# FireMines/zk_stark_project

Hardware: NVIDIA B200
Metric: stark_proofs_per_sec (higher is better)
Workload: dtype u128 mod p (f128 field, 4x u32 limbs), u32 BLAKE3

## Files before the change

### zk_stark_project_b200/csrc/kernels.cuh

```cuda
#pragma once
#include "f128.cuh"
#include "blake3.cuh"
#include "coin.cuh"

namespace zkb {

struct PowTab {
    const fe* lo;
    const fe* hi;
    uint32_t l1;
};
__device__ __forceinline__ fe powtab(const PowTab& t, uint32_t e) {
    fe a = fe_ldg(t.lo + (e & ((1u << t.l1) - 1u)));
    fe b = fe_ldg(t.hi + (e >> t.l1));
    return fe_mul(a, b);
}

struct LdeMat {
    fe* data;
    uint32_t log_n, log_beta, w, log_p;
    uint32_t log_shard, bw, bw_magic, view, q_self;
    uint64_t blk_stride;
    uint32_t k0, log_kc;
};
__device__ __forceinline__ uint32_t lde_full_log_p(const LdeMat& m) { return m.log_p + m.log_shard; }
__device__ __forceinline__ size_t lde_row_base(const LdeMat& m, uint32_t k, uint32_t i) {
    const uint32_t lt = m.log_n - lde_full_log_p(m);
    const uint32_t t_low = i & ((1u << lt) - 1u), slot = i >> lt;
    const size_t panel = ((size_t)(k - m.k0) << lt) + t_low;
    const size_t np = (size_t)1 << (m.log_kc + lt);
    const uint32_t chunk = m.view == 0 ? (slot >> m.log_p) : 0u;
    return (((size_t)chunk * np + panel) * m.bw << m.log_p) + (slot & ((1u << m.log_p) - 1u));
}
__device__ __forceinline__ size_t lde_col_off(const LdeMat& m, uint32_t j) {
    const uint32_t blk = (j * m.bw_magic) >> 16;
    return (size_t)blk * m.blk_stride + ((size_t)(j - blk * m.bw) << m.log_p);
}
__device__ __forceinline__ size_t lde_addr(const LdeMat& m, uint32_t k, uint32_t i, uint32_t j) {
    return lde_row_base(m, k, i) + lde_col_off(m, j);
}

__global__ void k_transpose_cols(const fe* __restrict__ in, fe* __restrict__ out, uint32_t n, uint32_t wc, uint32_t out_stride) {
    __shared__ uint4 tile[32][33];
    const uint32_t i0 = blockIdx.x * 32, j0 = blockIdx.y * 32;
    for (uint32_t jj = threadIdx.y; jj < 32; jj += blockDim.y) {
        uint32_t j = j0 + jj, i = i0 + threadIdx.x;
        if (j < wc && i < n) {
            const fe v = fe_canon(fe_load(in + (size_t)j * n + i), 0);
            tile[jj][threadIdx.x] = make_uint4(v.x[0], v.x[1], v.x[2], v.x[3]);
        }
    }
    __syncthreads();
    for (uint32_t ii = threadIdx.y; ii < 32; ii += blockDim.y) {
        uint32_t i = i0 + ii, j = j0 + threadIdx.x;
        if (j < wc && i < n) reinterpret_cast<uint4*>(out)[(size_t)i * out_stride + j] = tile[threadIdx.x][ii];
    }
}

struct NttPass {
    const fe* in;
    fe* out;
    uint32_t log_n, a, b;
    uint32_t w_in, w_out;
    uint32_t col0_in, col0_out, ncols, cj;
    uint32_t n_cosets, coset0;
    uint64_t in_coset_stride, out_coset_stride;
    uint32_t coset;
    uint32_t inverse;
    uint32_t log_tab;
    uint32_t log_lde;
    uint32_t out_panel;
    uint32_t log_shard;
    uint32_t panel_k0, log_kc;
    uint32_t do_scale;
    fe scale;
    PowTab roots;
    const fe* pow3;
    const fe* tw_tab;
};

__device__ __forceinline__ uint32_t bitrev(uint32_t v, uint32_t bits) { return bits == 0 ? 0u : (__brev(v) >> (32 - bits)); }

template <int RHO, int NC>
__device__ __forceinline__ void ntt_unit(fe* __restrict__ col, const uint32_t rs, const uint32_t cstride, const fe4* __restrict__ tw,
                                         const uint32_t base, const uint32_t lam0) {
    constexpr int R = 1 << RHO;
    fe x[NC][R];
    const uint32_t step = rs << lam0;
    fe* p = col + base * rs;
#pragma unroll
    for (int c = 0; c < NC; c++)
#pragma unroll
        for (int d = 0; d < R; d++) x[c][d] = p[d * step + c * cstride];
    const uint32_t base_low = base & ((1u << lam0) - 1u);
#pragma unroll
    for (int s = 0; s < RHO; s++) {
        const fe4* twl = tw + ((1u << (lam0 + s)) - 1u) + base_low;
#pragma unroll
        for (int t = 0; t < (1 << s); t++) {
            const fe4 w = twl[(uint32_t)t << lam0];
#pragma unroll
            for (int g = 0; g < (R >> (s + 1)); g++) {
                const int d0 = g * (2 << s) + t, d1 = d0 + (1 << s);
#pragma unroll
                for (int c = 0; c < NC; c++) {
                    const fe u = x[c][d0];
                    const fe v = fe_mul_pre4(x[c][d1], w);
                    x[c][d0] = fe_add(u, v);
                    x[c][d1] = fe_sub(u, v);
                }
            }
        }
    }
#pragma unroll
    for (int c = 0; c < NC; c++)
#pragma unroll
        for (int d = 0; d < R; d++) p[d * step + c * cstride] = x[c][d];
}

__device__ __forceinline__ fe ntt_twiddle(const NttPass& p, uint32_t k, uint32_t t_low, uint32_t q) {
    const uint32_t logS = p.b - p.a;
    const uint32_t tab_mask = (1u << p.log_tab) - 1u;
    const uint32_t lam = 32 - __clz(q + 1);
    const uint32_t th = q + 1 - (1u << (lam - 1));
    const uint32_t l = p.a + lam;
    (void)logS;
    uint32_t e = (t_low << (p.log_tab - l)) + (th << (p.log_tab - lam));
    if (p.coset) e += (k << (p.log_n - l)) << (p.log_tab - p.log_lde);
    e &= tab_mask;
    if (p.inverse) e = (0u - e) & tab_mask;
    fe t = powtab(p.roots, e);
    if (p.coset) t = fe_mul(t, fe_ldg(p.pow3 + l));
    return t;
}
__global__ void k_build_twiddles(const NttPass p, fe* __restrict__ table) {
    const uint32_t S = 1u << (p.b - p.a);
    const uint64_t total = ((uint64_t)p.n_cosets << p.a) * (S - 1u);
    const uint64_t id = (uint64_t)blockIdx.x * blockDim.x + threadIdx.x;
    if (id >= total) return;
    const uint32_t q = (uint32_t)(id % (S - 1u));
    const uint32_t tile = (uint32_t)(id / (S - 1u));
    fe_store(table + id, ntt_twiddle(p, tile >> p.a, tile & ((1u << p.a) - 1u), q));
}

template <int RHO>
__device__ __forceinline__ void ntt_unit_plain(fe* __restrict__ col, const uint32_t rs, const fe* __restrict__ tw, const uint32_t base, const uint32_t lam0) {
    constexpr int R = 1 << RHO;
    fe x[R];
    const uint32_t step = rs << lam0;
    fe* p = col + base * rs;
#pragma unroll
    for (int d = 0; d < R; d++) x[d] = p[d * step];
    const uint32_t base_low = base & ((1u << lam0) - 1u);
#pragma unroll
    for (int s = 0; s < RHO; s++) {
        const fe* twl = tw + ((1u << (lam0 + s)) - 1u) + base_low;
#pragma unroll
        for (int t = 0; t < (1 << s); t++) {
            const fe w = twl[(uint32_t)t << lam0];
#pragma unroll
            for (int g = 0; g < (R >> (s + 1)); g++) {
                const int d0 = g * (2 << s) + t, d1 = d0 + (1 << s);
                const fe u = x[d0];
                const fe v = fe_mul(x[d1], w);
                x[d0] = fe_add(u, v);
                x[d1] = fe_sub(u, v);
            }
        }
    }
#pragma unroll
    for (int d = 0; d < R; d++) p[d * step] = x[d];
}
template <int RHO>
__device__ __forceinline__ void ntt_round_plain(fe* sm, const fe* tw, uint32_t rs, uint32_t log_cj, uint32_t logS, uint32_t lam0) {
    const uint32_t cj_mask = (1u << log_cj) - 1u;
    const uint32_t units = (1u << (logS - RHO)) << log_cj;
    for (uint32_t idx = threadIdx.x; idx < units; idx += blockDim.x) {
        const uint32_t jj = idx & cj_mask, u = idx >> log_cj;
        const uint32_t base = (u & ((1u << lam0) - 1u)) + ((u >> lam0) << (lam0 + RHO));
        ntt_unit_plain<RHO>(sm + jj, rs, tw, base, lam0);
    }
}
__device__ __forceinline__ void ntt_rounds_plain(fe* sm, const fe* tw, uint32_t rs, uint32_t log_cj, uint32_t logS) {
    for (uint32_t lam0 = 0; lam0 < logS;) {
        const uint32_t left = logS - lam0;
        if (left >= 3 && left != 4) { ntt_round_plain<3>(sm, tw, rs, log_cj, logS, lam0); lam0 += 3; }
        else if (left >= 2) { ntt_round_plain<2>(sm, tw, rs, log_cj, logS, lam0); lam0 += 2; }
        else { ntt_round_plain<1>(sm, tw, rs, log_cj, logS, lam0); lam0 += 1; }
        __syncthreads();
    }
}

template <int RHO, int NC>
__device__ __forceinline__ void ntt_round(fe* sm, const fe4* tw, uint32_t rs, uint32_t log_cj, uint32_t logS, uint32_t lam0) {
    const uint32_t log_cw = log_cj - (NC == 2 ? 1u : 0u);
    const uint32_t cw_mask = (1u << log_cw) - 1u;
    const uint32_t units = (1u << (logS - RHO)) << log_cw;
    for (uint32_t idx = threadIdx.x; idx < units; idx += blockDim.x) {
        const uint32_t jj = idx & cw_mask, u = idx >> log_cw;
        const uint32_t base = (u & ((1u << lam0) - 1u)) + ((u >> lam0) << (lam0 + RHO));
        ntt_unit<RHO, NC>(sm + jj, rs, 1u << log_cw, tw, base, lam0);
    }
}
template <int NC>
__device__ __forceinline__ void ntt_rounds(fe* sm, const fe4* tw, uint32_t rs, uint32_t log_cj, uint32_t logS) {
    for (uint32_t lam0 = 0; lam0 < logS;) {
        const uint32_t left = logS - lam0;
        if (left >= 3 && left != 4) { ntt_round<3, NC>(sm, tw, rs, log_cj, logS, lam0); lam0 += 3; }
        else if (left >= 2) { ntt_round<2, NC>(sm, tw, rs, log_cj, logS, lam0); lam0 += 2; }
        else { ntt_round<1, NC>(sm, tw, rs, log_cj, logS, lam0); lam0 += 1; }
        __syncthreads();
    }
}

template <bool PRE>
__global__ void __launch_bounds__(256, PRE ? 2 : 3) k_ntt_pass(const NttPass p) {
    extern __shared__ uint4 smem_raw[];
    fe* sm = reinterpret_cast<fe*>(smem_raw);
    const uint32_t logS = p.b - p.a, S = 1u << logS, cj = p.cj;
    const uint32_t log_cj = 31 - __clz(cj);
    const uint32_t rs = cj + (cj > 1 ? 1u : 0u);
    fe4* tw = reinterpret_cast<fe4*>(sm + (size_t)S * rs);
    fe* tw1 = sm + (size_t)S * rs;

    const uint32_t n_ct = (p.ncols + cj - 1) >> log_cj;
    uint32_t id = blockIdx.x;
    const uint32_t ct = id % n_ct; id /= n_ct;
    const uint32_t kk = id % p.n_cosets; id /= p.n_cosets;
    const uint32_t t_low = id & ((1u << p.a) - 1u);
    const uint32_t u0 = id >> p.a;
    const uint32_t k = p.coset0 + kk;
    const fe* in = p.in + (size_t)kk * p.in_coset_stride;
    fe* out = p.out + (size_t)kk * p.out_coset_stride;
    if (p.tw_tab) {
        const fe* t = p.tw_tab + ((size_t)(k << p.a) + t_low) * (S - 1u);
        for (uint32_t q = threadIdx.x; q + 1 < S; q += blockDim.x) { if (PRE) tw[q] = fe4_from(fe_ldg(t + q)); else tw1[q] = fe_ldg(t + q); }
    } else {
        for (uint32_t q = threadIdx.x; q + 1 < S; q += blockDim.x) {
            const fe w = ntt_twiddle(p, k, t_low, q);
            if (PRE) tw[q] = fe4_from(w); else tw1[q] = w;
        }
    }
    const uint32_t c_base = ct << log_cj;
    const uint32_t jj_t = threadIdx.x & (cj - 1u), v_t = threadIdx.x >> log_cj, dv = blockDim.x >> log_cj;
    const bool col_ok = c_base + jj_t < p.ncols;
    {
        const size_t vstride = ((size_t)p.w_in << (p.log_n - p.b)) << p.a;
        const fe* src = in + (((size_t)u0 << p.a) + t_low) * p.w_in + p.col0_in + c_base + jj_t + (size_t)v_t * vstride;
        const size_t dstride = (size_t)dv * vstride;
        fe* smc = sm + jj_t;
        const uint32_t brs = (32u - logS) & 31u;
        if (col_ok) {
            for (uint32_t v = v_t; v < S; v += dv, src += dstride) smc[(__brev(v) >> brs) * rs] = fe_load(src);
        } else {
            for (uint32_t v = v_t; v < S; v += dv) smc[(__brev(v) >> brs) * rs] = fe_zero();
        }
    }
    __syncthreads();
    if (PRE) { if (cj >= 16) ntt_rounds<2>(sm, tw, rs, log_cj, logS); else ntt_rounds<1>(sm, tw, rs, log_cj, logS); }
    else ntt_rounds_plain(sm, tw1, rs, log_cj, logS);
    if (p.out_panel) {
        const size_t panel = ((size_t)(k - p.panel_k0) << p.a) + t_low;
        const uint32_t lp = logS - p.log_shard;
        const size_t np = (size_t)1 << (p.log_kc + p.a);
        const size_t chunk_stride = (np * p.w_out) << lp;
        const uint32_t th0 = threadIdx.x & (S - 1u), jj0 = logS >= 8 ? 0u : (threadIdx.x >> logS), djj = logS >= 8 ? 1u : (blockDim.x >> logS);
        fe* colp = p.out + ((panel * p.w_out + p.col0_out + c_base + jj0) << lp);
        for (uint32_t jj = jj0; jj < cj && c_base + jj < p.ncols; jj += djj, colp += (size_t)djj << lp) {
            for (uint32_t th = (logS >= 8 ? threadIdx.x : th0); th < S; th += blockDim.x)
                fe_store(colp + (size_t)(th >> lp) * chunk_stride + (th & ((1u << lp) - 1u)), sm[th * rs + jj]);
        }
    } else {
        const size_t tstride = (size_t)p.w_out << p.a;
        fe* dst = out + (((size_t)u0 << p.b) + t_low) * p.w_out + p.col0_out + c_base + jj_t + (size_t)v_t * tstride;
        const size_t dstride = (size_t)dv * tstride;
        const fe* smc = sm + jj_t;
        if (col_ok) {
            for (uint32_t th = v_t; th < S; th += dv, dst += dstride) {
                fe x = smc[th * rs];
                if (p.do_scale) x = fe_mul(x, p.scale);
                fe_store(dst, x);
            }
        }
    }
}

__global__ void k_scale_pow(fe* x, uint64_t n, PowTab base, fe scale, uint64_t keep, uint32_t* __restrict__ bad_degree) {
    uint64_t m = (uint64_t)blockIdx.x * blockDim.x + threadIdx.x;
    if (m >= n) return;
    const fe v = fe_load(x + m);
    if (m >= keep) { if (!fe_is_zero(v)) atomicOr(bad_degree, 1u); return; }
    fe f = fe_mul(powtab(base, (uint32_t)m), scale);
    fe_store(x + m, fe_mul(v, f));
}

__global__ void __launch_bounds__(128) k_hash_lde_rows(const LdeMat m, uint32_t* __restrict__ leaves, uint64_t leaf0, uint32_t compact) {
    const uint64_t gid = (uint64_t)blockIdx.x * blockDim.x + threadIdx.x;
    const uint32_t lpf = lde_full_log_p(m), lt = m.log_n - lpf;
    const uint32_t log_rows = m.log_kc + lt + (m.view == 0 ? lpf : m.log_p);
    if (gid >> log_rows) return;
    const uint32_t lslots = m.view == 0 ? lpf : m.log_p;
    const uint32_t s = (uint32_t)gid & ((1u << lslots) - 1u);
    const uint32_t panel = (uint32_t)(gid >> lslots);
    const uint32_t slot = m.view == 0 ? s : ((m.q_self << m.log_p) + s);
    const uint32_t k = m.k0 + (panel >> lt), t_low = panel & ((1u << lt) - 1u);
    const uint32_t i = t_low + (slot << lt);
    const uint64_t r = compact ? (((uint64_t)i << m.log_kc) + (k - m.k0)) : (((uint64_t)i << m.log_beta) + k - leaf0);
    uint32_t d[8];
    b3_hash_elems(m.data + lde_row_base(m, k, i), (size_t)1 << m.log_p, m.w, d, m.bw, m.bw_magic, m.blk_stride);
    uint4* o = reinterpret_cast<uint4*>(leaves + r * 8);
    o[0] = make_uint4(d[0], d[1], d[2], d[3]);
    o[1] = make_uint4(d[4], d[5], d[6], d[7]);
}
__global__ void __launch_bounds__(128) k_hash_lde_rows_split(const LdeMat m, uint32_t* __restrict__ leaves, uint64_t leaf0, uint32_t compact) {
    const uint64_t t = (uint64_t)blockIdx.x * blockDim.x + threadIdx.x;
    const uint32_t c = (uint32_t)t & 3u;
    const uint32_t lpf = lde_full_log_p(m), lt = m.log_n - lpf;
    const uint32_t log_rows = m.log_kc + lt + (m.view == 0 ? lpf : m.log_p);
    const bool live = ((t >> 2) >> log_rows) == 0;
    const uint64_t gid = live ? (t >> 2) : 0;
    const uint32_t lslots = m.view == 0 ? lpf : m.log_p;
    const uint32_t s = (uint32_t)gid & ((1u << lslots) - 1u);
    const uint32_t panel = (uint32_t)(gid >> lslots);
    const uint32_t slot = m.view == 0 ? s : ((m.q_self << m.log_p) + s);
    const uint32_t k = m.k0 + (panel >> lt), t_low = panel & ((1u << lt) - 1u);
    const uint32_t i = t_low + (slot << lt);
    const uint64_t r = compact ? (((uint64_t)i << m.log_kc) + (k - m.k0)) : (((uint64_t)i << m.log_beta) + k - leaf0);
    const uint32_t nchunks = (m.w + 63u) / 64u;
    uint32_t cv[8], nb[8];
    if (c < nchunks) b3_chunk_cv_elems(m.data + lde_row_base(m, k, i), (size_t)1 << m.log_p, m.w, c, cv, m.bw, m.bw_magic, m.blk_stride);
    else {
#pragma unroll
        for (int q = 0; q < 8; q++) cv[q] = 0;
    }
#pragma unroll
    for (int q = 0; q < 8; q++) nb[q] = __shfl_down_sync(0xffffffffu, cv[q], 1);
    if (c == 0 || (c == 2 && nchunks == 4)) {
        uint32_t o[8];
        b3_parent(cv, nb, nchunks == 2, o);
#pragma unroll
        for (int q = 0; q < 8; q++) cv[q] = o[q];
    }
    if (nchunks > 2) {
#pragma unroll
        for (int q = 0; q < 8; q++) nb[q] = __shfl_down_sync(0xffffffffu, cv[q], 2);
        if (c == 0) {
            uint32_t o[8];
            b3_parent(cv, nb, true, o);
#pragma unroll
            for (int q = 0; q < 8; q++) cv[q] = o[q];
        }
    }
    if (live && c == 0) {
        uint4* o = reinterpret_cast<uint4*>(leaves + r * 8);
        o[0] = make_uint4(cv[0], cv[1], cv[2], cv[3]);
        o[1] = make_uint4(cv[4], cv[5], cv[6], cv[7]);
    }
}
__global__ void k_permute_coset_items(const uint32_t* __restrict__ gathered, uint32_t* __restrict__ out, uint32_t log_n, uint32_t log_beta,
                                      uint32_t log_kc, uint32_t words) {
    const uint64_t t = (uint64_t)blockIdx.x * blockDim.x + threadIdx.x;
    const uint32_t q4 = words >> 2;
    const uint64_t item = t / q4;
    if (item >> (log_n + log_beta)) return;
    const uint32_t part = (uint32_t)(t - item * q4);
    const uint32_t k = (uint32_t)item & ((1u << log_beta) - 1u);
    const uint64_t i = item >> log_beta;
    const uint32_t src = k >> log_kc, kl = k & ((1u << log_kc) - 1u);
    const uint64_t from = ((uint64_t)src << (log_n + log_kc)) + (i << log_kc) + kl;
    reinterpret_cast<uint4*>(out)[item * q4 + part] = reinterpret_cast<const uint4*>(gathered)[from * q4 + part];
}

__global__ void __launch_bounds__(128) k_hash_strided_rows(const fe* __restrict__ e, uint64_t rows, uint32_t count, uint32_t* __restrict__ leaves) {
    const uint64_t i = (uint64_t)blockIdx.x * blockDim.x + threadIdx.x;
    if (i >= rows) return;
    uint32_t d[8];
    b3_hash_elems(e + i, rows, count, d, 256, 256, 0);
    uint4* o = reinterpret_cast<uint4*>(leaves + i * 8);
    o[0] = make_uint4(d[0], d[1], d[2], d[3]);
    o[1] = make_uint4(d[4], d[5], d[6], d[7]);
}

__global__ void __launch_bounds__(256) k_merkle_level(const uint32_t* __restrict__ src, uint32_t* __restrict__ dst, uint64_t count) {
    const uint64_t i = (uint64_t)blockIdx.x * blockDim.x + threadIdx.x;
    if (i >= count) return;
    const uint4* s = reinterpret_cast<const uint4*>(src + i * 16);
    uint32_t m[16], cv[8];
    uint4 a = s[0], b = s[1], c = s[2], d = s[3];
    m[0] = a.x; m[1] = a.y; m[2] = a.z; m[3] = a.w; m[4] = b.x; m[5] = b.y; m[6] = b.z; m[7] = b.w;
    m[8] = c.x; m[9] = c.y; m[10] = c.z; m[11] = c.w; m[12] = d.x; m[13] = d.y; m[14] = d.z; m[15] = d.w;
    b3_iv(cv);
    b3_compress(cv, m, 0, 64, B3_CHUNK_START | B3_CHUNK_END | B3_ROOT);
    uint4* o = reinterpret_cast<uint4*>(dst + i * 8);
    o[0] = make_uint4(cv[0], cv[1], cv[2], cv[3]);
    o[1] = make_uint4(cv[4], cv[5], cv[6], cv[7]);
}

__global__ void __launch_bounds__(512) k_merkle_top(uint32_t* __restrict__ heap, uint32_t top) {
    const uint32_t one_flags = B3_CHUNK_START | B3_CHUNK_END | B3_ROOT;
    for (uint32_t lvl = top; lvl >= 1; lvl >>= 1) {
        const uint32_t i = threadIdx.x;
        if (i < lvl) {
            const uint4* s = reinterpret_cast<const uint4*>(heap + (size_t)(2 * (lvl + i)) * 8);
            uint32_t m[16], cv[8];
            uint4 a = s[0], b = s[1], c = s[2], d = s[3];
            m[0] = a.x; m[1] = a.y; m[2] = a.z; m[3] = a.w; m[4] = b.x; m[5] = b.y; m[6] = b.z; m[7] = b.w;
            m[8] = c.x; m[9] = c.y; m[10] = c.z; m[11] = c.w; m[12] = d.x; m[13] = d.y; m[14] = d.z; m[15] = d.w;
            b3_iv(cv);
            b3_compress(cv, m, 0, 64, one_flags);
            uint4* o = reinterpret_cast<uint4*>(heap + (size_t)(lvl + i) * 8);
            o[0] = make_uint4(cv[0], cv[1], cv[2], cv[3]);
            o[1] = make_uint4(cv[4], cv[5], cv[6], cv[7]);
        }
        __threadfence_block();
        __syncthreads();
    }
}

enum { ZKB_AIR_TRAINING = 1, ZKB_AIR_AGGREGATION = 2, ZKB_AIR_MIMC = 3 };
#define ZKB_MAX_GROUPS 4
struct EvalParams {
    LdeMat lde;
    uint32_t air_id, log_ce;
    uint32_t n_trans;
    const fe* tcoef;
    uint32_t n_groups;
    uint32_t g_off[ZKB_MAX_GROUPS + 1];
    const uint32_t* a_col;
    const uint32_t* a_sel;
    const fe* a_val;
    const fe* a_coef;
    const fe* div;
    const fe* params;
    const fe* periodic;
// ... 523 lines not shown
```

### zk_stark_project_b200/csrc/zkb200.cu

```cuda
#include <cuda_runtime.h>
#include <dlfcn.h>
#include <sys/random.h>
#include <nccl.h>
#include <atomic>
#include <chrono>
#include <cstdio>
#include <cstdlib>
#include <functional>
#include <map>
#include <thread>
#include <tuple>
#include <memory>
#include "kernels.cuh"
#include "host.hpp"

namespace zkb {

struct CudaError : std::runtime_error { using std::runtime_error::runtime_error; };
struct StateError : std::runtime_error { using std::runtime_error::runtime_error; };

#define CK(call)                                                                                              \
    do {                                                                                                      \
        cudaError_t e_ = (call);                                                                              \
        if (e_ != cudaSuccess)                                                                                \
// ... 103 lines not shown
    const fe* d_aval() const { return d_in.as<fe>(); }
    const fe* d_params() const { return d_in.as<fe>() + air.assertions.size(); }
    DevBuf d_lde_rows, d_mg_a, d_mg_b;
    DevBuf d_cap;

    void count() { launches++; }
    static uint32_t magic16(uint32_t d) { return (65536u + d - 1) / d; }
    LdeMat std_mat(fe* data, uint32_t w, uint32_t log_p) const { return LdeMat{data, log_n, log_beta, w, log_p, 0, w, magic16(w), 0, 0, 0, 0, log_beta}; }
    bool mg_coset() const { return mg_active && (uint32_t)mg_world <= air.blowup; }
    uint32_t mg_log_kc() const { return log_beta - log_g; }
    LdeMat coset_mat(fe* data, uint32_t w, uint32_t log_p) const {
        LdeMat m = std_mat(data, w, log_p);
        if (mg_coset()) { m.log_kc = mg_log_kc(); m.k0 = (uint32_t)mg_rank << m.log_kc; }
        return m;
    }
    LdeMat lde_mat() const {
        if (!mg_active) return std_mat(d_lde.as<fe>(), air.w, lde_log_p);
        const uint32_t wl = air.w / (uint32_t)mg_world;
        return LdeMat{d_lde.as<fe>(), log_n, log_beta, wl, lde_log_p - log_g, log_g, wl, magic16(wl), 0, (uint32_t)mg_rank, 0, 0, log_beta};
    }
    LdeMat lde_rows_mat() const {
        const uint32_t wl = air.w / (uint32_t)mg_world, lp = lde_log_p - log_g;
        const uint64_t np = (uint64_t)1 << (log_beta + log_n - lde_log_p);
        return LdeMat{d_lde_rows.as<fe>(), log_n, log_beta, air.w, lp, log_g, wl, magic16(wl), 1, (uint32_t)mg_rank, (np * wl) << lp, 0, log_beta};
    }
    LdeMat comp_mat() const { return coset_mat(d_comp_lde.as<fe>(), c, comp_log_p); }
    LdeMat ab_mat() const { return coset_mat(d_ab_lde.as<fe>(), 2, ab_log_p); }

    void init(int dev, void* strm) {
        int ndev = 0;
        cudaError_t e = cudaGetDeviceCount(&ndev);
        if (e != cudaSuccess || ndev == 0) throw CudaError(std::string("no CUDA device available: ") + cudaGetErrorString(e));
        if (dev < 0 || dev >= ndev) throw InvalidArg("device index out of range");
        device = dev;
        CK(cudaSetDevice(device));
        stream = (cudaStream_t)strm;
        cudaDeviceProp prop;
        CK(cudaGetDeviceProperties(&prop, device));
        sm_count = prop.multiProcessorCount;
        CK(cudaFuncSetAttribute(k_ntt_pass<true>, cudaFuncAttributeMaxDynamicSharedMemorySize, 200 * 1024));
        CK(cudaFuncSetAttribute(k_ntt_pass<false>, cudaFuncAttributeMaxDynamicSharedMemorySize, 200 * 1024));
        for (auto& pr : tev) for (auto& x : pr) CK(cudaEventCreate(&x));
        h_stage_cap = (size_t)8 << 20;
        CK(cudaHostAlloc((void**)&h_stage, h_stage_cap, cudaHostAllocDefault));
        for (auto& x : ev_group) CK(cudaEventCreateWithFlags(&x, cudaEventDisableTiming));
        CK(cudaEventCreateWithFlags(&ev_done, cudaEventBlockingSync | cudaEventDisableTiming));
        CK(cudaStreamCreateWithFlags(&copy_stream, cudaStreamNonBlocking));
        {
            int lo = 0, hi = 0;
            CK(cudaDeviceGetStreamPriorityRange(&lo, &hi));
            CK(cudaStreamCreateWithPriority(&xchg_stream, cudaStreamNonBlocking, hi));
        }
        ev_ok = true;
        memset(&times, 0, sizeof(times));
    }
    void destroy() {
        cudaSetDevice(device);
        cudaStreamSynchronize(stream);
        for (DevBuf* b : {&d_trace, &d_bufA, &d_bufB, &d_tmp1, &d_tmp2, &d_lde, &d_tree, &d_small, &d_comp_evals, &d_comp_lde, &d_comp_tree,
                          &d_ab, &d_ab_lde, &d_deep, &d_roots_lo, &d_roots_hi, &d_inv3_lo, &d_inv3_hi, &d_pow3, &d_aux, &d_gather, &d_user_trace, &d_flags,
                          &d_lde_rows, &d_mg_a, &d_mg_b, &d_cap, &d_bnd_coef, &d_bnd_lde, &d_fs, &d_in, &d_rem_coef})
            b->release();
        if (comm) { g_nccl.CommDestroy(comm); comm = nullptr; }
        for (auto& b : d_fri_evals) b.release();
        for (auto& b : d_fri_tree) b.release();
        for (auto& kv : tw_cache) kv.second.release();
        for (auto& kv : pack_cache) kv.second.release();
        for (auto& kv : div_cache) kv.second.release();
        for (auto& kv : graphs) if (kv.second.exec) cudaGraphExecDestroy(kv.second.exec);
        if (ev_ok) { for (auto& pr : tev) for (auto& x : pr) cudaEventDestroy(x); for (auto& x : ev_group) cudaEventDestroy(x); cudaStreamDestroy(copy_stream); cudaStreamDestroy(xchg_stream); }
        if (h_stage) cudaFreeHost(h_stage);
        if (h_out) cudaFreeHost(h_out);
        if (ev_done) cudaEventDestroy(ev_done);
        if (owns_stream && stream) { cudaStreamDestroy(stream); stream = nullptr; }
    }

    void h2d(void* dst, const void* src, size_t bytes) { CK(cudaMemcpyAsync(dst, src, bytes, cudaMemcpyHostToDevice, stream)); }
    void h2d_small(void* dst, const void* src, size_t bytes) {
        if (bytes == 0) return;
        const size_t need = (bytes + 255) & ~(size_t)255;
        if (h_stage_used + need > h_stage_cap) {
            CK(cudaMemcpyAsync(dst, src, bytes, cudaMemcpyHostToDevice, stream));
            CK(cudaStreamSynchronize(stream));
            return;
        }
        memcpy(h_stage + h_stage_used, src, bytes);
        CK(cudaMemcpyAsync(dst, h_stage + h_stage_used, bytes, cudaMemcpyHostToDevice, stream));
        h_stage_used += need;
    }
    void t_begin(int st) { if (!capturing) CK(cudaEventRecord(tev[st][0], stream)); }
    void t_end(int st) { if (!capturing) { CK(cudaEventRecord(tev[st][1], stream)); trec[st] = true; times_valid = false; } }
    void collect_times() {
        if (times_valid) return;
        CK(cudaSetDevice(device));
        CK(cudaStreamSynchronize(stream));
        float* slot[TS_COUNT] = {&times.lde, &times.interpolate, &times.leaf_hash, &times.merkle, &times.constraints, &times.composition,
                                 &times.ood, &times.deep, &times.fri, &times.grind, &times.queries, &times.total};
        for (int st = 0; st < TS_COUNT; st++) if (trec[st]) CK(cudaEventElapsedTime(slot[st], tev[st][0], tev[st][1]));
        times_valid = true;
    }
    void d2h(void* dst, const void* src, size_t bytes) {
        CK(cudaMemcpyAsync(dst, src, bytes, cudaMemcpyDeviceToHost, stream));
        CK(cudaStreamSynchronize(stream));
    }
    void check_launch() { CK(cudaGetLastError()); count(); }

    static void build_powtab(HF base, uint32_t log_size, std::vector<HF>& lo, std::vector<HF>& hi, uint32_t& l1) {
        l1 = (log_size + 1) / 2;
        uint32_t l2 = log_size - l1;
        lo.resize((size_t)1 << l1); hi.resize((size_t)1 << l2);
        HF x = HF::raw(1);
        for (auto& v : lo) { v = x; x = x * base; }
        HF step = x;
        x = HF::raw(1);
        for (auto& v : hi) { v = x; x = x * step; }
    }
    void ensure_tables() {
        if (tab_log_built != log_N) {
            std::vector<HF> lo, hi; uint32_t l1;
            build_powtab(HF::root_of_unity(log_N), log_N, lo, hi, l1);
            d_roots_lo.ensure(lo.size() * 16); d_roots_hi.ensure(hi.size() * 16);
            h2d(d_roots_lo.p, lo.data(), lo.size() * 16); h2d(d_roots_hi.p, hi.data(), hi.size() * 16);
            roots = PowTab{d_roots_lo.as<fe>(), d_roots_hi.as<fe>(), l1};
            build_powtab(HF::from_u64(3).inv(), log_N, lo, hi, l1);
            d_inv3_lo.ensure(lo.size() * 16); d_inv3_hi.ensure(hi.size() * 16);
            h2d(d_inv3_lo.p, lo.data(), lo.size() * 16); h2d(d_inv3_hi.p, hi.data(), hi.size() * 16);
            inv3tab = PowTab{d_inv3_lo.as<fe>(), d_inv3_hi.as<fe>(), l1};
            CK(cudaStreamSynchronize(stream));
            tab_log_built = log_N;
            pow3_for_log_n = 0;
        }
        log_tab = log_N;
        if (pow3_for_log_n != log_n) {
            std::vector<HF> p3(log_n + 1);
            for (uint32_t l = 0; l <= log_n; l++) p3[l] = HF::from_u64(3).pow((u128)(air.n >> l));
            d_pow3.ensure(64 * 16);
            h2d(d_pow3.p, p3.data(), p3.size() * 16);
            CK(cudaStreamSynchronize(stream));
            pow3_for_log_n = log_n;
        }
    }

    static uint32_t pick_cj(uint32_t ncols) { return ncols >= 9 ? 16 : ncols >= 5 ? 8 : ncols >= 3 ? 4 : ncols == 2 ? 2 : 1; }
    static bool pre_twiddles(uint32_t cj) { return cj >= 4; }
    static std::vector<uint32_t> plan_layers(uint32_t log_len, uint32_t cj) {
        uint32_t maxlog = pre_twiddles(cj) ? (cj >= 16 ? 8 : 9) : 12 - log2u(cj);
        uint32_t passes = (log_len + maxlog - 1) / maxlog;
        if (passes == 0) passes = 1;
        std::vector<uint32_t> b;
        uint32_t done = 0;
        for (uint32_t q = 0; q < passes; q++) { uint32_t take = (log_len - done + (passes - q) - 1) / (passes - q); done += take; b.push_back(done); }
        return b;
    }
    std::map<std::tuple<uint32_t, uint32_t, uint32_t, uint32_t, uint32_t, uint32_t>, DevBuf> tw_cache;
    size_t tw_cache_bytes = 0;
    const fe* twiddle_table(const NttPass& p, uint32_t all_cosets) {
        const uint32_t S = 1u << (p.b - p.a);
        const uint64_t entries = ((uint64_t)all_cosets << p.a) * (S - 1u), bytes = entries * 16;
        if (S < 2 || bytes > ((uint64_t)(pre_twiddles(p.cj) ? 64 : 192) << 20)) return nullptr;
        const auto key = std::make_tuple(p.log_n, p.a, p.b, p.coset, p.inverse, p.coset ? p.log_lde : 0u);
        auto it = tw_cache.find(key);
        if (it != tw_cache.end()) return it->second.as<fe>();
        if (tw_cache_bytes + bytes > ((uint64_t)768 << 20)) {
            CK(cudaStreamSynchronize(stream));
            for (auto& kv : tw_cache) kv.second.release();
            tw_cache.clear(); tw_cache_bytes = 0;
        }
        DevBuf& b = tw_cache[key];
        b.ensure(bytes);
        tw_cache_bytes += bytes;
        NttPass q = p;
        q.n_cosets = all_cosets; q.coset0 = 0; q.tw_tab = nullptr;
        k_build_twiddles<<<(unsigned)((entries + 255) / 256), 256, 0, stream>>>(q, b.as<fe>());
        check_launch();
        return b.as<fe>();
    }
    void launch_pass(NttPass& p) {
        const uint32_t S = 1u << (p.b - p.a);
        const uint32_t rs = p.cj + (p.cj > 1 ? 1 : 0);
        const bool pre = pre_twiddles(p.cj);
        const size_t smem = ((size_t)S * rs + (pre ? 4 : 1) * (size_t)S) * 16;
        const uint64_t tiles = (uint64_t)((p.ncols + p.cj - 1) / p.cj) * p.n_cosets * ((uint64_t)1 << (p.log_n - (p.b - p.a)));
        if (tiles > 0x7fffffffull) throw InvalidArg("transform too large for one launch");
        if (pre) {
            const uint32_t units = p.cj >= 16 ? S * p.cj / 16 : S * p.cj / 8;
            uint32_t threads = std::max<uint32_t>(units, std::min<uint32_t>(S, 256));
            threads = std::min<uint32_t>(256, std::max<uint32_t>(32, threads));
            k_ntt_pass<true><<<(unsigned)tiles, threads, smem, stream>>>(p);
        } else k_ntt_pass<false><<<(unsigned)tiles, 256, smem, stream>>>(p);
        check_launch();
    }
    struct Xform {
        const fe* in; uint32_t w_in, col0_in;
        fe* out; uint32_t w_out, col0_out;
        uint32_t ncols, log_len;
        bool inverse, coset_lde;
        uint32_t log_lde;
        bool scale; HF scale_by;
        uint32_t log_shard = 0;
        uint32_t coset_lo = 0, coset_cnt = 0;
        uint32_t batch_cosets = 0;
        std::function<void(uint32_t, uint32_t)> after_batch;
        uint32_t cj = 0;
    };
    uint32_t run_xform(const Xform& x, DevBuf& s1, DevBuf& s2) {
        const uint32_t cj = x.cj ? x.cj : pick_cj(x.ncols);
        std::vector<uint32_t> bnd = plan_layers(x.log_len, cj);
        const uint32_t passes = (uint32_t)bnd.size();
        const uint64_t len = (uint64_t)1 << x.log_len;
        const uint32_t all_cosets = x.coset_lde ? (1u << (x.log_lde - x.log_len)) : 1;
        const uint32_t n_cosets = (x.coset_lde && x.coset_cnt) ? x.coset_cnt : all_cosets;
        uint32_t batch = x.batch_cosets ? std::min(x.batch_cosets, n_cosets) : n_cosets;
        if (passes > 1) {
            const uint64_t per = len * x.ncols * 16;
            uint64_t budget = (uint64_t)6 << 30;
            batch = (uint32_t)std::max<uint64_t>(1, std::min<uint64_t>(batch, budget / std::max<uint64_t>(per, 1)));
            s1.ensure(per * batch);
            if (passes > 2) s2.ensure(per * batch);
        }
        for (uint32_t k0 = 0; k0 < n_cosets; k0 += batch) {
            const uint32_t nk = std::min(batch, n_cosets - k0);
            uint32_t a = 0;
            const fe* src = x.in; uint32_t w_src = x.w_in, c0_src = x.col0_in; uint64_t src_stride = 0;
            for (uint32_t q = 0; q < passes; q++) {
                NttPass p{};
                const bool last = (q + 1 == passes);
                p.in = src; p.w_in = w_src; p.col0_in = c0_src; p.in_coset_stride = src_stride;
                p.log_n = x.log_len; p.a = a; p.b = bnd[q];
                p.ncols = x.ncols; p.cj = cj; p.n_cosets = nk; p.coset0 = x.coset_lo + k0;
                p.panel_k0 = x.coset_lo; p.log_kc = log2u(n_cosets);
                p.coset = x.coset_lde ? 1 : 0; p.inverse = x.inverse ? 1 : 0;
                p.log_tab = log_tab; p.log_lde = x.coset_lde ? x.log_lde : 0;
                p.roots = roots; p.pow3 = d_pow3.as<fe>();
                p.tw_tab = twiddle_table(p, all_cosets);
                if (last) {
                    p.out = x.out; p.w_out = x.w_out; p.col0_out = x.col0_out;
                    p.out_panel = x.coset_lde ? 1 : 0;
                    p.log_shard = x.coset_lde ? x.log_shard : 0;
                    if (p.log_shard > p.b - p.a) throw InvalidArg("trace too short to shard its LDE panels across this many GPUs");
                    p.out_coset_stride = 0;
                    p.do_scale = x.scale ? 1 : 0; p.scale = to_fe(x.scale_by);
                } else {
                    fe* dst = (q % 2 == 0) ? s1.as<fe>() : s2.as<fe>();
                    p.out = dst; p.w_out = x.ncols; p.col0_out = 0; p.out_coset_stride = len * x.ncols;
                    src = dst; w_src = x.ncols; c0_src = 0; src_stride = len * x.ncols;
                }
                launch_pass(p);
                a = bnd[q];
            }
            if (x.after_batch) x.after_batch(x.coset_lo + k0, nk);
        }
        return bnd.back() - (passes > 1 ? bnd[passes - 2] : 0);
    }

    void build_merkle(uint32_t* heap, uint64_t n_leaves) {
        uint64_t lvl = n_leaves / 2;
        for (; lvl > 512; lvl >>= 1) {
            k_merkle_level<<<(unsigned)((lvl + 255) / 256), 256, 0, stream>>>(heap + 2 * lvl * 8, heap + lvl * 8, lvl);
            check_launch();
        }
        k_merkle_top<<<1, 512, 0, stream>>>(heap, (uint32_t)lvl);
        check_launch();
    }

    void begin(const zkb_air_desc* desc) {
        CK(cudaSetDevice(device));
        air = AirSpec::from_desc(desc);
        log_n = log2u(air.n); log_beta = log2u(air.blowup); log_N = log_n + log_beta;
        log_ce = log2u(air.ce_blowup()); c = air.num_comp_cols();
        if ((1u << log_ce) > air.blowup) throw InvalidArg("constraint evaluation blowup exceeds the LDE blowup");
        {
            std::set<uint64_t> steps;
            for (auto& a : air.assertions) steps.insert(a.step);
            if (steps.size() > ZKB_MAX_GROUPS) throw InvalidArg("too many distinct assertion steps (boundary groups)");
        }
        ensure_tables();
        parts = ProofParts();
        memset(&ts, 0, sizeof(ts));
        ts.comp_degree_ok = 1;
        memset(&times, 0, sizeof(times));
        for (auto& r : trec) r = false;
        times_valid = true;
        h_stage_used = 0;
        coin.init(air.coin_seed());
        fri_layers = air.num_fri_layers();
        if (fri_layers > 16) throw InvalidArg("too many FRI layers");
        fri_layer = 0; fri_committed = false;
        positions.clear();
        mg_active = false;
        {
            auto al = [](size_t x) { return (x + 255) & ~(size_t)255; };
            const uint32_t w = air.w, q = air.num_queries;
            const uint64_t m_last = air.lde_size() >> (4 * fri_layers);
            fs = FsLayout();
            fs.o_ood = al(sizeof(DevTs));
            fs.o_rem = fs.o_ood + (2 * (size_t)w + c) * 16;
            fs.rem_cap = (uint32_t)std::max<uint64_t>(1, m_last / air.blowup);
            size_t off = al(fs.o_rem + (size_t)fs.rem_cap * 16);
            auto add_tree = [&](uint32_t width, uint32_t depth) {
                FsTree t{off, off + (size_t)q * width * 16, width, depth};
                off = al(t.o_paths + (size_t)q * depth * 32);
                fs.trees.push_back(t);
            };
            add_tree(w, log_N);
            add_tree(c, log_N);
            for (uint32_t l = 0; l < fri_layers; l++) add_tree(16, log2u(fri_domain(l) / 16));
            fs.host_bytes = off;
            fs.o_coef = off; off += ((size_t)air.num_transition() + air.assertions.size()) * 16;
            fs.o_gamma = off; off += ((size_t)w + c) * 16;
            fs.o_scr = off; off += 2 * (size_t)w * 16;
            fs.total = off;
            d_fs.ensure(fs.total);
            d_flags.ensure(256);
            if (h_out_cap < fs.host_bytes) {
                if (h_out) { cudaFreeHost(h_out); h_out = nullptr; h_out_cap = 0; }
                g_alloc_epoch++;
                CK(cudaHostAlloc((void**)&h_out, fs.host_bytes, cudaHostAllocDefault));
                h_out_cap = fs.host_bytes;
            }
            DevTs h0;
            memset(&h0, 0, sizeof(h0));
            memcpy(h0.seed, coin.seed, 32);
            h0.nonce = ~0ull;
            h2d_small(d_fs.p, &h0, sizeof(h0));
            const size_t na = air.assertions.size(), np = air.params.size();
            std::vector<HF> in(na + np);
            for (size_t i = 0; i < na; i++) in[i] = air.assertions[i].value;
            for (size_t i = 0; i < np; i++) in[na + i] = air.params[i];
            d_in.ensure((na + np + 1) * 16);
            h2d_small(d_in.p, in.data(), in.size() * 16);
        }
        stage = ST_BEGUN;
    }

    void trace_commit(const uint8_t* const* host_cols, const fe* d_src, uint8_t root_out[32]) {
        trace_commit_dev(host_cols, d_src);
        Digest32 root;
        d2h(root.b, d_tree.as<uint32_t>() + 8, 32);
        parts.commitments.push_back(root);
        memcpy(ts.trace_root, root.b, 32);
        if (root_out) memcpy(root_out, root.b, 32);
    }
    void trace_commit_dev(const uint8_t* const* host_cols, const fe* d_src) {
        if (stage != ST_BEGUN) throw StateError("zkb_trace_commit: call zkb_begin first");
        const uint64_t n = air.n, N = air.lde_size();
        const uint32_t w = air.w;
        std::vector<std::pair<uint32_t, uint32_t>> groups;
        if (!host_cols) groups.push_back({0, w});
        else for (uint32_t c0 = 0, step = 16; c0 < w; c0 += groups.back().second, step = std::min(step + 16, 48u)) groups.push_back({c0, std::min(step, w - c0)});
        const uint32_t ngroups = (uint32_t)groups.size();
        d_bufA.ensure(n * w * 16); d_bufB.ensure(n * w * 16);
        d_lde.ensure(N * w * 16);
        d_tree.ensure(2 * N * 32);
        t_begin(TS_LDE);
        if (host_cols) {
            d_trace.ensure((size_t)w * n * 16);
            for (uint32_t j = 0; j < w; j++) if (!host_cols[j]) throw InvalidArg("null trace column");
            CK(cudaEventRecord(ev_group[16], stream));
            CK(cudaStreamWaitEvent(copy_stream, ev_group[16], 0));
            if (ngroups > 16) throw InvalidArg("too many column groups");
            for (uint32_t g = 0; g < ngroups; g++) {
                const uint32_t c0 = groups[g].first, wc = groups[g].second;
                bool contiguous = true;
                for (uint32_t j = 1; j < wc; j++) if (host_cols[c0 + j] != host_cols[c0] + (size_t)j * n * 16) contiguous = false;
                uint8_t* dst = d_trace.as<uint8_t>() + (size_t)c0 * n * 16;
                if (contiguous) CK(cudaMemcpyAsync(dst, host_cols[c0], (size_t)wc * n * 16, cudaMemcpyHostToDevice, copy_stream));
                else for (uint32_t j = 0; j < wc; j++) CK(cudaMemcpyAsync(dst + (size_t)j * n * 16, host_cols[c0 + j], n * 16, cudaMemcpyHostToDevice, copy_stream));
                CK(cudaEventRecord(ev_group[g], copy_stream));
            }
            d_src = d_trace.as<fe>();
        }
        d_polys = d_bufB.as<fe>();
        const HF n_inv = HF::from_u64(n).inv();
        for (uint32_t g = 0; g < ngroups; g++) {
            const uint32_t c0 = groups[g].first, wc = groups[g].second;
            if (host_cols) CK(cudaStreamWaitEvent(stream, ev_group[g], 0));
            {
                dim3 grid((unsigned)((n + 31) / 32), (wc + 31) / 32), block(32, 8);
                k_transpose_cols<<<grid, block, 0, stream>>>(d_src + (size_t)c0 * n, d_bufA.as<fe>() + c0, (uint32_t)n, wc, w);
                check_launch();
            }
            Xform xi{d_bufA.as<fe>(), w, c0, d_bufB.as<fe>(), w, c0, wc, log_n, true, false, 0, true, n_inv};
            xi.cj = pick_cj(w);
            run_xform(xi, d_tmp1, d_tmp2);
            Xform xl{d_polys, w, c0, d_lde.as<fe>(), w, c0, wc, log_n, false, true, log_N, false, HF()};
            xl.cj = pick_cj(w);
            lde_log_p = run_xform(xl, d_tmp1, d_tmp2);
// ... 1173 lines not shown
```

Measured before the change: 77.13.

## Precompute four-copy twiddle tables and load via cp.async; use 3D grid

Twiddle tables for pre-expanded passes are now stored in four-copy (fe4) form and copied into shared memory with cp.async, so the async load overlaps the global-to-shared tile load. The 1D block index with div/mod decoding becomes a 3D grid, chunked along z to stay under the dimension limit. The load and store loops get trip counts computed up front with partial unrolling, and the common cj=16, logS=8 case gets a hardcoded round schedule. In exchange, the four-copy tables take four times the memory, which may trigger more cache eviction, and a host-side logging env var is added.

```diff
diff --git a/zk_stark_project_b200/csrc/kernels.cuh b/zk_stark_project_b200/csrc/kernels.cuh
--- a/zk_stark_project_b200/csrc/kernels.cuh
+++ b/zk_stark_project_b200/csrc/kernels.cuh
@@ -77,6 +77,8 @@
     PowTab roots;
     const fe* pow3;
     const fe* tw_tab;
+    uint32_t tw_four;
+    uint32_t tile0;
 };
 
 __device__ __forceinline__ uint32_t bitrev(uint32_t v, uint32_t bits) { return bits == 0 ? 0u : (__brev(v) >> (32 - bits)); }
@@ -140,7 +142,15 @@
     if (id >= total) return;
     const uint32_t q = (uint32_t)(id % (S - 1u));
     const uint32_t tile = (uint32_t)(id / (S - 1u));
-    fe_store(table + id, ntt_twiddle(p, tile >> p.a, tile & ((1u << p.a) - 1u), q));
+    const fe w = ntt_twiddle(p, tile >> p.a, tile & ((1u << p.a) - 1u), q);
+    if (p.tw_four) {
+        const fe4 t = fe4_from(w);
+#pragma unroll
+        for (int i = 0; i < 4; i++) fe_store(table + 4 * id + i, t.w[i]);
+    } else fe_store(table + id, w);
+}
+__device__ __forceinline__ void cp_async16(void* smem_dst, const void* gmem_src) {
+    asm volatile("cp.async.cg.shared.global [%0], [%1], 16;" ::"r"((uint32_t)__cvta_generic_to_shared(smem_dst)), "l"(gmem_src) : "memory");
 }
 
 template <int RHO>
@@ -204,6 +214,14 @@
 }
 template <int NC>
 __device__ __forceinline__ void ntt_rounds(fe* sm, const fe4* tw, uint32_t rs, uint32_t log_cj, uint32_t logS) {
+    if (NC == 2 && log_cj == 4 && logS == 8) {
+        uint32_t lam0 = 0;
+        asm("" : "+r"(lam0));
+        ntt_round<3, NC>(sm, tw, 17, 4, 8, lam0); __syncthreads();
+        ntt_round<3, NC>(sm, tw, 17, 4, 8, 3); __syncthreads();
+        ntt_round<2, NC>(sm, tw, 17, 4, 8, 6); __syncthreads();
+        return;
+    }
     for (uint32_t lam0 = 0; lam0 < logS;) {
         const uint32_t left = logS - lam0;
         if (left >= 3 && left != 4) { ntt_round<3, NC>(sm, tw, rs, log_cj, logS, lam0); lam0 += 3; }
@@ -223,39 +241,46 @@
     fe4* tw = reinterpret_cast<fe4*>(sm + (size_t)S * rs);
     fe* tw1 = sm + (size_t)S * rs;
 
-    const uint32_t n_ct = (p.ncols + cj - 1) >> log_cj;
-    uint32_t id = blockIdx.x;
-    const uint32_t ct = id % n_ct; id /= n_ct;
-    const uint32_t kk = id % p.n_cosets; id /= p.n_cosets;
+    const uint32_t ct = blockIdx.x, kk = blockIdx.y, id = p.tile0 + blockIdx.z;
     const uint32_t t_low = id & ((1u << p.a) - 1u);
     const uint32_t u0 = id >> p.a;
     const uint32_t k = p.coset0 + kk;
-    const fe* in = p.in + (size_t)kk * p.in_coset_stride;
-    fe* out = p.out + (size_t)kk * p.out_coset_stride;
-    if (p.tw_tab) {
-        const fe* t = p.tw_tab + ((size_t)(k << p.a) + t_low) * (S - 1u);
-        for (uint32_t q = threadIdx.x; q + 1 < S; q += blockDim.x) { if (PRE) tw[q] = fe4_from(fe_ldg(t + q)); else tw1[q] = fe_ldg(t + q); }
+    if (PRE && p.tw_four) {
+        const uint4* t = reinterpret_cast<const uint4*>(p.tw_tab) + ((size_t)(k << p.a) + t_low) * (4u * (S - 1u));
+        uint4* d = reinterpret_cast<uint4*>(tw);
+#pragma unroll 1
+        for (uint32_t q = threadIdx.x; q < 4u * (S - 1u); q += blockDim.x) cp_async16(d + q, t + q);
+        asm volatile("cp.async.commit_group;" ::: "memory");
     } else {
+        const fe* t = p.tw_tab ? p.tw_tab + ((size_t)(k << p.a) + t_low) * (S - 1u) : nullptr;
         for (uint32_t q = threadIdx.x; q + 1 < S; q += blockDim.x) {
-            const fe w = ntt_twiddle(p, k, t_low, q);
+            const fe w = t ? fe_ldg(t + q) : ntt_twiddle(p, k, t_low, q);
             if (PRE) tw[q] = fe4_from(w); else tw1[q] = w;
         }
     }
     const uint32_t c_base = ct << log_cj;
-    const uint32_t jj_t = threadIdx.x & (cj - 1u), v_t = threadIdx.x >> log_cj, dv = blockDim.x >> log_cj;
+    const uint32_t log_bd = 31 - __clz(blockDim.x), log_dv = log_bd - log_cj;
+    const uint32_t jj_t = threadIdx.x & (cj - 1u), v_t = threadIdx.x >> log_cj, dv = 1u << log_dv;
+    const uint32_t nrow = v_t < S ? ((S - 1u - v_t) >> log_dv) + 1u : 0u;
     const bool col_ok = c_base + jj_t < p.ncols;
     {
         const size_t vstride = ((size_t)p.w_in << (p.log_n - p.b)) << p.a;
-        const fe* src = in + (((size_t)u0 << p.a) + t_low) * p.w_in + p.col0_in + c_base + jj_t + (size_t)v_t * vstride;
+        const fe* src = p.in + (size_t)kk * p.in_coset_stride + (((size_t)u0 << p.a) + t_low) * p.w_in + p.col0_in + c_base + jj_t +
+                        (size_t)v_t * vstride;
         const size_t dstride = (size_t)dv * vstride;
-        fe* smc = sm + jj_t;
+        char* smc = reinterpret_cast<char*>(sm + jj_t);
         const uint32_t brs = (32u - logS) & 31u;
+        const uint32_t rs16 = rs * 16u;
+        uint32_t vs = v_t << brs;
+        const uint32_t dvs = dv << brs;
         if (col_ok) {
-            for (uint32_t v = v_t; v < S; v += dv, src += dstride) smc[(__brev(v) >> brs) * rs] = fe_load(src);
+#pragma unroll 4
+            for (uint32_t i = 0; i < nrow; i++, vs += dvs, src += dstride) *reinterpret_cast<fe*>(smc + __brev(vs) * rs16) = fe_load(src);
         } else {
-            for (uint32_t v = v_t; v < S; v += dv) smc[(__brev(v) >> brs) * rs] = fe_zero();
-        }
-    }
+            for (uint32_t i = 0; i < nrow; i++, vs += dvs) *reinterpret_cast<fe*>(smc + __brev(vs) * rs16) = fe_zero();
+        }
+    }
+    if (PRE) asm volatile("cp.async.wait_all;" ::: "memory");
     __syncthreads();
     if (PRE) { if (cj >= 16) ntt_rounds<2>(sm, tw, rs, log_cj, logS); else ntt_rounds<1>(sm, tw, rs, log_cj, logS); }
     else ntt_rounds_plain(sm, tw1, rs, log_cj, logS);
@@ -264,22 +289,33 @@
         const uint32_t lp = logS - p.log_shard;
         const size_t np = (size_t)1 << (p.log_kc + p.a);
         const size_t chunk_stride = (np * p.w_out) << lp;
-        const uint32_t th0 = threadIdx.x & (S - 1u), jj0 = logS >= 8 ? 0u : (threadIdx.x >> logS), djj = logS >= 8 ? 1u : (blockDim.x >> logS);
+        const bool wide = S >= blockDim.x;
+        const uint32_t th0 = wide ? threadIdx.x : (threadIdx.x & (S - 1u)), dth = wide ? blockDim.x : S;
+        const uint32_t jj0 = wide ? 0u : (threadIdx.x >> logS), log_djj = wide ? 0u : log_bd - logS, djj = 1u << log_djj;
+        const uint32_t jend = min(cj, p.ncols - c_base);
+        const uint32_t ncol = jj0 < jend ? ((jend - 1u - jj0) >> log_djj) + 1u : 0u;
+        const size_t cstep = (size_t)djj << lp;
         fe* colp = p.out + ((panel * p.w_out + p.col0_out + c_base + jj0) << lp);
-        for (uint32_t jj = jj0; jj < cj && c_base + jj < p.ncols; jj += djj, colp += (size_t)djj << lp) {
-            for (uint32_t th = (logS >= 8 ? threadIdx.x : th0); th < S; th += blockDim.x)
-                fe_store(colp + (size_t)(th >> lp) * chunk_stride + (th & ((1u << lp) - 1u)), sm[th * rs + jj]);
+#pragma unroll 1
+        for (uint32_t th = th0; th < S; th += dth) {
+            fe* d = colp + (size_t)(th >> lp) * chunk_stride + (th & ((1u << lp) - 1u));
+            const fe* s = sm + th * rs + jj0;
+#pragma unroll 4
+            for (uint32_t j = 0; j < ncol; j++, d += cstep, s += djj) fe_store(d, *s);
         }
     } else {
         const size_t tstride = (size_t)p.w_out << p.a;
-        fe* dst = out + (((size_t)u0 << p.b) + t_low) * p.w_out + p.col0_out + c_base + jj_t + (size_t)v_t * tstride;
+        fe* dst = p.out + (size_t)kk * p.out_coset_stride + (((size_t)u0 << p.b) + t_low) * p.w_out + p.col0_out + c_base + jj_t +
+                  (size_t)v_t * tstride;
         const size_t dstride = (size_t)dv * tstride;
-        const fe* smc = sm + jj_t;
+        const fe* s = sm + v_t * rs + jj_t;
+        const uint32_t sstep = dv * rs;
         if (col_ok) {
-            for (uint32_t th = v_t; th < S; th += dv, dst += dstride) {
-                fe x = smc[th * rs];
-                if (p.do_scale) x = fe_mul(x, p.scale);
-                fe_store(dst, x);
+            if (p.do_scale) {
+                for (uint32_t i = 0; i < nrow; i++, dst += dstride, s += sstep) fe_store(dst, fe_mul(*s, p.scale));
+            } else {
+#pragma unroll 4
+                for (uint32_t i = 0; i < nrow; i++, dst += dstride, s += sstep) fe_store(dst, *s);
             }
         }
     }
diff --git a/zk_stark_project_b200/csrc/zkb200.cu b/zk_stark_project_b200/csrc/zkb200.cu
--- a/zk_stark_project_b200/csrc/zkb200.cu
+++ b/zk_stark_project_b200/csrc/zkb200.cu
@@ -279,43 +279,67 @@
         for (uint32_t q = 0; q < passes; q++) { uint32_t take = (log_len - done + (passes - q) - 1) / (passes - q); done += take; b.push_back(done); }
         return b;
     }
-    std::map<std::tuple<uint32_t, uint32_t, uint32_t, uint32_t, uint32_t, uint32_t>, DevBuf> tw_cache;
+    std::map<std::tuple<uint32_t, uint32_t, uint32_t, uint32_t, uint32_t, uint32_t, uint32_t>, DevBuf> tw_cache;
     size_t tw_cache_bytes = 0;
-    const fe* twiddle_table(const NttPass& p, uint32_t all_cosets) {
+    void twiddle_table(NttPass& p, uint32_t all_cosets) {
         const uint32_t S = 1u << (p.b - p.a);
-        const uint64_t entries = ((uint64_t)all_cosets << p.a) * (S - 1u), bytes = entries * 16;
-        if (S < 2 || bytes > ((uint64_t)(pre_twiddles(p.cj) ? 64 : 192) << 20)) return nullptr;
-        const auto key = std::make_tuple(p.log_n, p.a, p.b, p.coset, p.inverse, p.coset ? p.log_lde : 0u);
+        const uint64_t entries = ((uint64_t)all_cosets << p.a) * (S - 1u);
+        const bool pre = pre_twiddles(p.cj);
+        const uint64_t cap = (uint64_t)(pre ? 64 : 192) << 20;
+        p.tw_tab = nullptr; p.tw_four = 0;
+        static const bool log_tables = getenv("ZKB_HOST_PROFILE") != nullptr;
+        if (S < 2 || entries * 16 > cap) {
+            if (log_tables && S >= 2)
+                fprintf(stderr, "[zkb twiddles] log_n %u layers [%u, %u) coset %u inverse %u cj %u: no table (%.2f MiB plain), generated\n", p.log_n,
+                        p.a, p.b, p.coset, p.inverse, p.cj, entries * 16 / 1048576.0);
+            return;
+        }
+        const uint32_t four = pre && entries * 64 <= cap ? 1u : 0u;
+        const uint64_t bytes = entries * (four ? 64 : 16);
+        const auto key = std::make_tuple(p.log_n, p.a, p.b, p.coset, p.inverse, p.coset ? p.log_lde : 0u, four);
         auto it = tw_cache.find(key);
-        if (it != tw_cache.end()) return it->second.as<fe>();
-        if (tw_cache_bytes + bytes > ((uint64_t)768 << 20)) {
-            CK(cudaStreamSynchronize(stream));
-            for (auto& kv : tw_cache) kv.second.release();
-            tw_cache.clear(); tw_cache_bytes = 0;
-        }
-        DevBuf& b = tw_cache[key];
-        b.ensure(bytes);
-        tw_cache_bytes += bytes;
-        NttPass q = p;
-        q.n_cosets = all_cosets; q.coset0 = 0; q.tw_tab = nullptr;
-        k_build_twiddles<<<(unsigned)((entries + 255) / 256), 256, 0, stream>>>(q, b.as<fe>());
-        check_launch();
-        return b.as<fe>();
-    }
-    void launch_pass(NttPass& p) {
+        if (it == tw_cache.end()) {
+            if (tw_cache_bytes + bytes > ((uint64_t)768 << 20)) {
+                if (log_tables) fprintf(stderr, "[zkb twiddles] cache of %.2f MiB over budget: cleared\n", tw_cache_bytes / 1048576.0);
+                CK(cudaStreamSynchronize(stream));
+                for (auto& kv : tw_cache) kv.second.release();
+                tw_cache.clear(); tw_cache_bytes = 0;
+            }
+            DevBuf& b = tw_cache[key];
+            b.ensure(bytes);
+            tw_cache_bytes += bytes;
+            if (log_tables)
+                fprintf(stderr, "[zkb twiddles] log_n %u layers [%u, %u) coset %u inverse %u cj %u: %s table %.2f MiB, cache %.2f MiB\n", p.log_n, p.a,
+                        p.b, p.coset, p.inverse, p.cj, four ? "four-copy" : "plain", bytes / 1048576.0, tw_cache_bytes / 1048576.0);
+            NttPass q = p;
+            q.n_cosets = all_cosets; q.coset0 = 0; q.tw_four = four;
+            k_build_twiddles<<<(unsigned)((entries + 255) / 256), 256, 0, stream>>>(q, b.as<fe>());
+            check_launch();
+            it = tw_cache.find(key);
+        }
+        p.tw_tab = it->second.as<fe>(); p.tw_four = four;
+    }
+    void launch_pass(NttPass p) {
         const uint32_t S = 1u << (p.b - p.a);
         const uint32_t rs = p.cj + (p.cj > 1 ? 1 : 0);
         const bool pre = pre_twiddles(p.cj);
         const size_t smem = ((size_t)S * rs + (pre ? 4 : 1) * (size_t)S) * 16;
-        const uint64_t tiles = (uint64_t)((p.ncols + p.cj - 1) / p.cj) * p.n_cosets * ((uint64_t)1 << (p.log_n - (p.b - p.a)));
-        if (tiles > 0x7fffffffull) throw InvalidArg("transform too large for one launch");
+        const uint32_t n_ct = (p.ncols + p.cj - 1) / p.cj;
+        const uint64_t tiles = (uint64_t)1 << (p.log_n - (p.b - p.a));
+        if (p.n_cosets > 65535) throw InvalidArg("transform too large for one launch");
+        uint32_t threads = 256;
         if (pre) {
             const uint32_t units = p.cj >= 16 ? S * p.cj / 16 : S * p.cj / 8;
-            uint32_t threads = std::max<uint32_t>(units, std::min<uint32_t>(S, 256));
+            threads = std::max<uint32_t>(units, std::min<uint32_t>(S, 256));
             threads = std::min<uint32_t>(256, std::max<uint32_t>(32, threads));
-            k_ntt_pass<true><<<(unsigned)tiles, threads, smem, stream>>>(p);
-        } else k_ntt_pass<false><<<(unsigned)tiles, 256, smem, stream>>>(p);
-        check_launch();
+        }
+        for (uint64_t z0 = 0; z0 < tiles; z0 += 65535) {
+            p.tile0 = (uint32_t)z0;
+            const dim3 grid(n_ct, p.n_cosets, (unsigned)std::min<uint64_t>(65535, tiles - z0));
+            if (pre) k_ntt_pass<true><<<grid, threads, smem, stream>>>(p);
+            else k_ntt_pass<false><<<grid, threads, smem, stream>>>(p);
+            check_launch();
+        }
     }
     struct Xform {
         const fe* in; uint32_t w_in, col0_in;
@@ -359,7 +383,7 @@
                 p.coset = x.coset_lde ? 1 : 0; p.inverse = x.inverse ? 1 : 0;
                 p.log_tab = log_tab; p.log_lde = x.coset_lde ? x.log_lde : 0;
                 p.roots = roots; p.pow3 = d_pow3.as<fe>();
-                p.tw_tab = twiddle_table(p, all_cosets);
+                twiddle_table(p, all_cosets);
                 if (last) {
                     p.out = x.out; p.w_out = x.w_out; p.col0_out = x.col0_out;
                     p.out_panel = x.coset_lde ? 1 : 0;
```

Measured after the change: 82.08, median of 6. 1.06x the previous value.
